# A-SHOJAEI/adverse-weather-semantic-segmentation-robustness-benchmark

Measured on AMD Instinct MI355X. Metric: images/sec (1024x2048, 5 weather conds, ensemble eval), higher is better.
Workload: dtype f32 (results float32; attention, gemm_1x1, winograd_3x3, segformer_head on 3xf16 split operands: 22-bit operands, f32 accumulate)

## Files before the change

### adverse_weather_semantic_segmentation_robustness_benchmark_amd/csrc/attn.hip

```cpp
#include "awseg_common.h"

namespace {

typedef float f32x16 __attribute__((ext_vector_type(16)));

constexpr int AT = 256;
#ifndef AWSEG_ATTN_SPLIT_WAVES
#define AWSEG_ATTN_SPLIT_WAVES 2
#endif
constexpr int D = 32;
constexpr int TK = 32;
constexpr int LDK = 36;

__device__ __forceinline__ constexpr int acc_row(int r, int hk) { return (r & 3) + 8 * (r >> 2) + 4 * hk; }

__global__ __launch_bounds__(AT, 2)
void attention_d32_kernel(const float* __restrict__ q, const float* __restrict__ k, const float* __restrict__ v,
                          float* __restrict__ out, int nq, int nkv, int heads, float scale_log2e, int kvp)
{
    __shared__ float sK[2][TK * LDK];
    __shared__ float sV[2][D * LDK];
    const int tid = threadIdx.x, lane = tid & 63, wave = tid >> 6;
    const int hk = lane >> 5, li = lane & 31;
    const int h = blockIdx.y, b = blockIdx.z;
    const int C = heads * D;
    const int q0 = blockIdx.x * 128 + wave * 32;
    const float* kb = k + (size_t)b * nkv * kvp + h * D;
    const float* vb = v + (size_t)b * nkv * kvp + h * D;

    float qf[16];
    {
        const int qi = q0 + li;
        const float* qp = q + ((size_t)b * nq + (qi < nq ? qi : nq - 1)) * C + h * D;
#pragma unroll
        for (int s4 = 0; s4 < 8; ++s4) {
            const float4 t4 = *reinterpret_cast<const float4*>(qp + 4 * s4);
            qf[2 * s4] = (hk ? t4.y : t4.x) * scale_log2e;
            qf[2 * s4 + 1] = (hk ? t4.w : t4.z) * scale_log2e;
        }
    }
    const int lkey = tid >> 3, lc = tid & 7;
    const size_t g_off = (size_t)lkey * kvp + 4 * lc;
    const int wk0 = lkey * LDK + 2 * lc;
    const int vkk = (lkey >> 2) & 1, vr = (lkey & 3) + 4 * (lkey >> 3);
    const int wv0 = (4 * lc) * LDK + vkk * 16 + vr;
    auto stage = [&](int buf, const float4& kk4, const float4& vv4) {
        *reinterpret_cast<float2*>(&sK[buf][wk0]) = make_float2(kk4.x, kk4.z);
        *reinterpret_cast<float2*>(&sK[buf][wk0 + 16]) = make_float2(kk4.y, kk4.w);
        sV[buf][wv0] = vv4.x; sV[buf][wv0 + LDK] = vv4.y; sV[buf][wv0 + 2 * LDK] = vv4.z; sV[buf][wv0 + 3 * LDK] = vv4.w;
    };
    const int ntiles = nkv / TK;
    float4 kreg = *reinterpret_cast<const float4*>(kb + g_off), vreg = *reinterpret_cast<const float4*>(vb + g_off);
    stage(0, kreg, vreg);
    if (ntiles > 1) {
        kreg = *reinterpret_cast<const float4*>(kb + (size_t)TK * kvp + g_off);
        vreg = *reinterpret_cast<const float4*>(vb + (size_t)TK * kvp + g_off);
    }
    __syncthreads();

    f32x16 oacc;
#pragma unroll
    for (int r = 0; r < 16; ++r) oacc[r] = 0.f;
    float m_run = -1e30f, l_run = 0.f;
    const int a_off = li * LDK + hk * 16;

    for (int t = 0; t < ntiles; ++t) {
        const int buf = t & 1;
        float kf[16];
#pragma unroll
        for (int j = 0; j < 4; ++j) {
            const float4 t4 = *reinterpret_cast<const float4*>(&sK[buf][a_off + 4 * j]);
            kf[4 * j] = t4.x; kf[4 * j + 1] = t4.y; kf[4 * j + 2] = t4.z; kf[4 * j + 3] = t4.w;
        }
        f32x16 sacc;
#pragma unroll
        for (int r = 0; r < 16; ++r) sacc[r] = 0.f;
#pragma unroll
        for (int s = 0; s < 16; ++s) sacc = __builtin_amdgcn_mfma_f32_32x32x2f32(kf[s], qf[s], sacc, 0, 0, 0);
        float vf[16];
#pragma unroll
        for (int j = 0; j < 4; ++j) {
            const float4 t4 = *reinterpret_cast<const float4*>(&sV[buf][a_off + 4 * j]);
            vf[4 * j] = t4.x; vf[4 * j + 1] = t4.y; vf[4 * j + 2] = t4.z; vf[4 * j + 3] = t4.w;
        }
        float mt = fmaxf(fmaxf(sacc[0], sacc[1]), fmaxf(sacc[2], sacc[3]));
#pragma unroll
        for (int r = 4; r < 16; r += 4) mt = fmaxf(mt, fmaxf(fmaxf(sacc[r], sacc[r + 1]), fmaxf(sacc[r + 2], sacc[r + 3])));
        mt = fmaxf(mt, __shfl_xor(mt, 32, 64));
        const float m_new = fmaxf(m_run, mt);
        const float alpha = __builtin_amdgcn_exp2f(m_run - m_new);
        float p[16], ls = 0.f;
#pragma unroll
        for (int r = 0; r < 16; ++r) { p[r] = __builtin_amdgcn_exp2f(sacc[r] - m_new); ls += p[r]; }
        ls += __shfl_xor(ls, 32, 64);
        l_run = l_run * alpha + ls;
        m_run = m_new;
        if (__builtin_amdgcn_ballot_w64(alpha != 1.0f) != 0) {
#pragma unroll
            for (int r = 0; r < 16; ++r) oacc[r] *= alpha;
        }
#pragma unroll
        for (int r = 0; r < 16; ++r) oacc = __builtin_amdgcn_mfma_f32_32x32x2f32(vf[r], p[r], oacc, 0, 0, 0);
        if (t + 1 < ntiles) {
            stage(buf ^ 1, kreg, vreg);
            if (t + 2 < ntiles) {
                kreg = *reinterpret_cast<const float4*>(kb + (size_t)(t + 2) * TK * kvp + g_off);
                vreg = *reinterpret_cast<const float4*>(vb + (size_t)(t + 2) * TK * kvp + g_off);
            }
        }
        __syncthreads();
    }

    const int qi = q0 + li;
    if (qi < nq) {
        const float inv = 1.0f / l_run;
        float* op = out + ((size_t)b * nq + qi) * C + h * D;
#pragma unroll
        for (int g = 0; g < 4; ++g)
            *reinterpret_cast<float4*>(op + 8 * g + 4 * hk) =
                make_float4(oacc[4 * g] * inv, oacc[4 * g + 1] * inv, oacc[4 * g + 2] * inv, oacc[4 * g + 3] * inv);
    }
}

typedef _Float16 h8 __attribute__((ext_vector_type(8)));
typedef _Float16 h2 __attribute__((ext_vector_type(2)));
typedef unsigned u32x4 __attribute__((ext_vector_type(4)));
typedef unsigned u32x2 __attribute__((ext_vector_type(2)));

constexpr int SROW = 72;
constexpr float kLoScale = 2048.0f, kLoInv = 1.0f / 2048.0f;

__device__ __forceinline__ void split_pair(float a, float b, unsigned& hi, unsigned& lo)
{
    const auto hp = __builtin_amdgcn_cvt_pkrtz(a, b);
    const h2 hh = __builtin_bit_cast(h2, hp);
    const float ra = (a - (float)hh.x) * kLoScale, rb = (b - (float)hh.y) * kLoScale;
    hi = __builtin_bit_cast(unsigned, hp);
    lo = __builtin_bit_cast(unsigned, __builtin_amdgcn_cvt_pkrtz(ra, rb));
}
__device__ __forceinline__ void split_pair_unscaled(float a, float b, unsigned& hi, unsigned& lo)
{
    hi = __builtin_bit_cast(unsigned, __builtin_amdgcn_cvt_pkrtz(a, b));
    asm("v_fma_mixlo_f16 %0, %1, 1.0, -%3 op_sel_hi:[0,0,1]\n\t"
        "v_fma_mixhi_f16 %0, %2, 1.0, -%3 op_sel:[0,0,1] op_sel_hi:[0,0,1]\n\t"
        "s_nop 1"
        : "=&v"(lo) : "v"(a), "v"(b), "v"(hi));
}
__device__ __forceinline__ void split8_unscaled(const float* x, h8& hi, h8& lo)
{
    u32x4 H, L;
#pragma unroll
    for (int i = 0; i < 4; ++i) { unsigned h, l; split_pair_unscaled(x[2 * i], x[2 * i + 1], h, l); H[i] = h; L[i] = l; }
    hi = __builtin_bit_cast(h8, H); lo = __builtin_bit_cast(h8, L);
}
__device__ __forceinline__ void split8(const float* x, h8& hi, h8& lo)
{
    u32x4 H, L;
#pragma unroll
    for (int i = 0; i < 4; ++i) { unsigned h, l; split_pair(x[2 * i], x[2 * i + 1], h, l); H[i] = h; L[i] = l; }
    hi = __builtin_bit_cast(h8, H); lo = __builtin_bit_cast(h8, L);
}
__device__ __forceinline__ constexpr int pv_slot(int key)
{
    return (key & 16) | (((key >> 2) & 1) << 3) | (((key >> 3) & 1) << 2) | (key & 3);
}

constexpr float kSplitLimit = 32768.0f;
struct attn_scales { float sq, sk, sv, bq, bk, bv; };

__device__ __forceinline__ float amax4(float m, const float4& t)
{
    m = __builtin_fmaxf(__builtin_fmaxf(m, __builtin_fabsf(t.x)), __builtin_fabsf(t.y));
    return __builtin_fmaxf(__builtin_fmaxf(m, __builtin_fabsf(t.z)), __builtin_fabsf(t.w));
}

typedef __bf16 bf8 __attribute__((ext_vector_type(8)));
__device__ __forceinline__ unsigned pack_bf16(float a, float b)
{
    typedef __bf16 bf2 __attribute__((ext_vector_type(2)));
    typedef float f2 __attribute__((ext_vector_type(2)));
    return __builtin_bit_cast(unsigned, __builtin_convertvector(f2{a, b}, bf2));
}
__device__ __forceinline__ h8 pack8_bf16(const float* x)
{
    u32x4 H;
#pragma unroll
    for (int i = 0; i < 4; ++i) H[i] = pack_bf16(x[2 * i], x[2 * i + 1]);
    return __builtin_bit_cast(h8, H);
}
#define MFMA_BF(A, B, C) __builtin_amdgcn_mfma_f32_32x32x16_bf16(__builtin_bit_cast(bf8, A), __builtin_bit_cast(bf8, B), C, 0, 0, 0)

template <bool SCALED, bool BF16 = false>
__device__ __forceinline__ bool attn_split_pass(const float* __restrict__ q, const float* __restrict__ k, const float* __restrict__ v,
                                                float* __restrict__ out, int nq, int nkv, int heads, float scale_log2e, int kvp,
                                                _Float16 (*sK)[TK * SROW], _Float16 (*sV)[D * SROW], unsigned* sMax, const attn_scales sc)
{
    const int tid = threadIdx.x, lane = tid & 63, wave = tid >> 6;
    const int hk = lane >> 5, li = lane & 31;
    const int h = blockIdx.y, b = blockIdx.z;
    const int C = heads * D;
    const int q0 = blockIdx.x * 128 + wave * 32;
    const float* kb = k + (size_t)b * nkv * kvp + h * D;
    const float* vb = v + (size_t)b * nkv * kvp + h * D;
    float qmax = 0.f, kmax = 0.f, vmax = 0.f;

    h8 qh[2], ql[2];
    {
        const int qi = q0 + li;
        const float* qp = q + ((size_t)b * nq + (qi < nq ? qi : nq - 1)) * C + h * D;
        const float qs = SCALED ? scale_log2e * sc.sq : scale_log2e;
#pragma unroll
        for (int s = 0; s < 2; ++s) {
            const float4 a4 = *reinterpret_cast<const float4*>(qp + 16 * s + 8 * hk);
            const float4 b4 = *reinterpret_cast<const float4*>(qp + 16 * s + 8 * hk + 4);
            const float x[8] = { a4.x * qs, a4.y * qs, a4.z * qs, a4.w * qs, b4.x * qs, b4.y * qs, b4.z * qs, b4.w * qs };
            if (BF16) { qh[s] = pack8_bf16(x); continue; }
            if (!SCALED) {
#pragma unroll
                for (int i = 0; i < 8; ++i) qmax = __builtin_fmaxf(qmax, __builtin_fabsf(x[i]));
            }
            split8(x, qh[s], ql[s]);
        }
    }
    const int lkey = tid >> 3, lc = tid & 7;
    const size_t g_off = (size_t)lkey * kvp + 4 * lc;
    const int wk0 = lkey * SROW + 4 * lc;
    const int wv0 = (4 * lc) * SROW + pv_slot(lkey);
    auto stage = [&](int buf, float4 kk4, float4 vv4) {
        if (BF16) {
            u32x2 H;
            H[0] = pack_bf16(kk4.x, kk4.y); H[1] = pack_bf16(kk4.z, kk4.w);
            *reinterpret_cast<u32x2*>(&sK[buf][wk0]) = H;
            const unsigned v01 = pack_bf16(vv4.x, vv4.y), v23 = pack_bf16(vv4.z, vv4.w);
            unsigned short* svb = reinterpret_cast<unsigned short*>(&sV[buf][wv0]);
            svb[0] = (unsigned short)v01; svb[SROW] = (unsigned short)(v01 >> 16);
            svb[2 * SROW] = (unsigned short)v23; svb[3 * SROW] = (unsigned short)(v23 >> 16);
            return;
        }
        if (SCALED) {
            kk4.x *= sc.sk; kk4.y *= sc.sk; kk4.z *= sc.sk; kk4.w *= sc.sk;
            vv4.x *= sc.sv; vv4.y *= sc.sv; vv4.z *= sc.sv; vv4.w *= sc.sv;
        } else {
            kmax = amax4(kmax, kk4); vmax = amax4(vmax, vv4);
        }
        u32x2 H, L; unsigned hh, ll;
        split_pair(kk4.x, kk4.y, hh, ll); H[0] = hh; L[0] = ll;
        split_pair(kk4.z, kk4.w, hh, ll); H[1] = hh; L[1] = ll;
        *reinterpret_cast<u32x2*>(&sK[buf][wk0]) = H;
        *reinterpret_cast<u32x2*>(&sK[buf][wk0 + 32]) = L;
        unsigned vh01, vl01, vh23, vl23;
        split_pair(vv4.x, vv4.y, vh01, vl01);
        split_pair(vv4.z, vv4.w, vh23, vl23);
        unsigned short* sv = reinterpret_cast<unsigned short*>(&sV[buf][wv0]);
        sv[0] = (unsigned short)vh01;            sv[32] = (unsigned short)vl01;
        sv[SROW] = (unsigned short)(vh01 >> 16); sv[SROW + 32] = (unsigned short)(vl01 >> 16);
        sv[2 * SROW] = (unsigned short)vh23;     sv[2 * SROW + 32] = (unsigned short)vl23;
        sv[3 * SROW] = (unsigned short)(vh23 >> 16); sv[3 * SROW + 32] = (unsigned short)(vl23 >> 16);
    };
    const int ntiles = nkv / TK;
    float4 kreg = *reinterpret_cast<const float4*>(kb + g_off), vreg = *reinterpret_cast<const float4*>(vb + g_off);
    stage(0, kreg, vreg);
    if (ntiles > 1) {
        kreg = *reinterpret_cast<const float4*>(kb + (size_t)TK * kvp + g_off);
        vreg = *reinterpret_cast<const float4*>(vb + (size_t)TK * kvp + g_off);
    }
    __syncthreads();

    f32x16 om, oc;
#pragma unroll
    for (int r = 0; r < 16; ++r) { om[r] = 0.f; oc[r] = 0.f; }
    float m_run = -1e30f, l_run = 0.f;
    const int a_off = li * SROW + 8 * hk;

    for (int t = 0; t < ntiles; ++t) {
        const int buf = t & 1;
        const h8* kr = reinterpret_cast<const h8*>(&sK[buf][a_off]);
        const h8 kh0 = kr[0], kh1 = kr[2], kl0 = kr[4], kl1 = kr[6];
        f32x16 sm, scx;
#pragma unroll
        for (int r = 0; r < 16; ++r) { sm[r] = 0.f; scx[r] = 0.f; }
        if (BF16) {
            sm = MFMA_BF(kh0, qh[0], sm);
            sm = MFMA_BF(kh1, qh[1], sm);
        } else {
            sm = __builtin_amdgcn_mfma_f32_32x32x16_f16(kh0, qh[0], sm, 0, 0, 0);
            scx = __builtin_amdgcn_mfma_f32_32x32x16_f16(kh0, ql[0], scx, 0, 0, 0);
            sm = __builtin_amdgcn_mfma_f32_32x32x16_f16(kh1, qh[1], sm, 0, 0, 0);
            scx = __builtin_amdgcn_mfma_f32_32x32x16_f16(kh1, ql[1], scx, 0, 0, 0);
            scx = __builtin_amdgcn_mfma_f32_32x32x16_f16(kl0, qh[0], scx, 0, 0, 0);
            scx = __builtin_amdgcn_mfma_f32_32x32x16_f16(kl1, qh[1], scx, 0, 0, 0);
        }
        const h8* vr = reinterpret_cast<const h8*>(&sV[buf][a_off]);
        const h8 vh0 = vr[0], vh1 = vr[2], vl0 = vr[4], vl1 = vr[6];
        float s[16];
#pragma unroll
        for (int r = 0; r < 16; ++r) {
            s[r] = fmaf(scx[r], kLoInv, sm[r]);
            if (SCALED) s[r] = s[r] * sc.bq * sc.bk;
        }
        float mt = fmaxf(fmaxf(s[0], s[1]), fmaxf(s[2], s[3]));
#pragma unroll
        for (int r = 4; r < 16; r += 4) mt = fmaxf(mt, fmaxf(fmaxf(s[r], s[r + 1]), fmaxf(s[r + 2], s[r + 3])));
        mt = fmaxf(mt, __shfl_xor(mt, 32, 64));
        const float m_new = fmaxf(m_run, mt);
        const float alpha = __builtin_amdgcn_exp2f(m_run - m_new);
        const float m_sh = m_new - 15.0f;
        float p[16], ls = 0.f;
#pragma unroll
        for (int r = 0; r < 16; ++r) { p[r] = __builtin_amdgcn_exp2f(s[r] - m_sh); ls += p[r]; }
        ls += __shfl_xor(ls, 32, 64);
        l_run = l_run * alpha + ls;
        m_run = m_new;
        if (__builtin_amdgcn_ballot_w64(alpha != 1.0f) != 0) {
#pragma unroll
            for (int r = 0; r < 16; ++r) { om[r] *= alpha; oc[r] *= alpha; }
        }
        if (BF16) {
            om = MFMA_BF(vh0, pack8_bf16(p), om);
            om = MFMA_BF(vh1, pack8_bf16(p + 8), om);
            if (t + 1 < ntiles) {
                stage(buf ^ 1, kreg, vreg);
                if (t + 2 < ntiles) {
                    kreg = *reinterpret_cast<const float4*>(kb + (size_t)(t + 2) * TK * kvp + g_off);
                    vreg = *reinterpret_cast<const float4*>(vb + (size_t)(t + 2) * TK * kvp + g_off);
                }
            }
            __syncthreads();
            continue;
        }
        h8 ph0, pl0, ph1, pl1;
        split8_unscaled(p, ph0, pl0);
        split8_unscaled(p + 8, ph1, pl1);
        om = __builtin_amdgcn_mfma_f32_32x32x16_f16(vh0, ph0, om, 0, 0, 0);
        oc = __builtin_amdgcn_mfma_f32_32x32x16_f16(vl0, ph0, oc, 0, 0, 0);
        om = __builtin_amdgcn_mfma_f32_32x32x16_f16(vh1, ph1, om, 0, 0, 0);
        oc = __builtin_amdgcn_mfma_f32_32x32x16_f16(vl1, ph1, oc, 0, 0, 0);
        om = __builtin_amdgcn_mfma_f32_32x32x16_f16(vh0, pl0, om, 0, 0, 0);
        om = __builtin_amdgcn_mfma_f32_32x32x16_f16(vh1, pl1, om, 0, 0, 0);
        if (t + 1 < ntiles) {
            stage(buf ^ 1, kreg, vreg);
            if (t + 2 < ntiles) {
                kreg = *reinterpret_cast<const float4*>(kb + (size_t)(t + 2) * TK * kvp + g_off);
                vreg = *reinterpret_cast<const float4*>(vb + (size_t)(t + 2) * TK * kvp + g_off);
            }
        }
        __syncthreads();
    }

    if (!SCALED && !BF16) {
        if (qmax >= kSplitLimit) atomicMax(&sMax[0], __builtin_bit_cast(unsigned, qmax));
        if (kmax >= kSplitLimit) atomicMax(&sMax[1], __builtin_bit_cast(unsigned, kmax));
        if (vmax >= kSplitLimit) atomicMax(&sMax[2], __builtin_bit_cast(unsigned, vmax));
        __syncthreads();
        if ((sMax[0] | sMax[1] | sMax[2]) != 0u) return true;
    }
    const int qi = q0 + li;
    if (qi < nq) {
        const float inv = 1.0f / l_run;
        float* op = out + ((size_t)b * nq + qi) * C + h * D;
#pragma unroll
        for (int g = 0; g < 4; ++g) {
            float4 o4 = make_float4(fmaf(oc[4 * g], kLoInv, om[4 * g]) * inv, fmaf(oc[4 * g + 1], kLoInv, om[4 * g + 1]) * inv,
                                    fmaf(oc[4 * g + 2], kLoInv, om[4 * g + 2]) * inv, fmaf(oc[4 * g + 3], kLoInv, om[4 * g + 3]) * inv);
            if (SCALED) { o4.x *= sc.bv; o4.y *= sc.bv; o4.z *= sc.bv; o4.w *= sc.bv; }
            *reinterpret_cast<float4*>(op + 8 * g + 4 * hk) = o4;
        }
    }
    return false;
}

__device__ __forceinline__ int guard_exponent(unsigned maxbits)
{
    const int ex = (int)(maxbits >> 23) & 0xff;
    if (maxbits == 0u || ex == 0xff) return 0;
    return ex - 127 - 13;
}

__global__ __launch_bounds__(AT, AWSEG_ATTN_SPLIT_WAVES)
void attention_d32_split_kernel(const float* __restrict__ q, const float* __restrict__ k, const float* __restrict__ v,
                                float* __restrict__ out, int nq, int nkv, int heads, float scale_log2e, int kvp)
{
    __shared__ __attribute__((aligned(16))) _Float16 sK[2][TK * SROW];
    __shared__ __attribute__((aligned(16))) _Float16 sV[2][D * SROW];
    __shared__ unsigned sMax[3];
    if (threadIdx.x < 3) sMax[threadIdx.x] = 0u;
    const attn_scales one = {1.f, 1.f, 1.f, 1.f, 1.f, 1.f};
    if (!attn_split_pass<false>(q, k, v, out, nq, nkv, heads, scale_log2e, kvp, sK, sV, sMax, one)) return;
    const int eq = guard_exponent(sMax[0]), ek = guard_exponent(sMax[1]), ev = guard_exponent(sMax[2]);
    auto p2 = [](int e) { return __builtin_bit_cast(float, (unsigned)(127 + e) << 23); };
    const attn_scales sc = {p2(-eq), p2(-ek), p2(-ev), p2(eq), p2(ek), p2(ev)};
    attn_split_pass<true>(q, k, v, out, nq, nkv, heads, scale_log2e, kvp, sK, sV, sMax, sc);
}

constexpr int IMG_TILE_HALFS = (TK + D) * SROW;

__device__ __forceinline__ uint32_t at_lds_addr(const void* p) { return (uint32_t)(uintptr_t)(__attribute__((address_space(3))) const void*)p; }
__device__ __forceinline__ void at_dma16(__amdgpu_buffer_rsrc_t rsrc, uint32_t voff, uint32_t soff, uint32_t lds_base)
{
    asm volatile("s_mov_b32 m0, %3\n\ts_nop 0\n\tbuffer_load_dwordx4 %0, %1, %2 offen lds" : : "v"(voff), "s"(rsrc), "s"(soff), "s"(lds_base) : "m0", "memory");
}

__global__ __launch_bounds__(AT)
void attn_kv_image_kernel(const float* __restrict__ k, const float* __restrict__ v, int kvp, int nkv, int heads,
                          _Float16* __restrict__ img, int* __restrict__ exps)
{
    __shared__ unsigned sM[2];
    const int tid = threadIdx.x, h = blockIdx.x, b = blockIdx.y;
    const float* kb = k + (size_t)b * nkv * kvp + h * D;
    const float* vb = v + (size_t)b * nkv * kvp + h * D;
    const int lkey = tid >> 3, lc = tid & 7;
    const size_t g_off = (size_t)lkey * kvp + 4 * lc;
    const int wk0 = lkey * SROW + 4 * lc;
    const int wv0 = TK * SROW + (4 * lc) * SROW + pv_slot(lkey);
    const int ntiles = nkv / TK;
    if (tid < 2) sM[tid] = 0u;
    __syncthreads();
    float kmax = 0.f, vmax = 0.f;
    for (int t = 0; t < ntiles; ++t) {
        kmax = amax4(kmax, *reinterpret_cast<const float4*>(kb + (size_t)t * TK * kvp + g_off));
        vmax = amax4(vmax, *reinterpret_cast<const float4*>(vb + (size_t)t * TK * kvp + g_off));
    }
    if (kmax >= kSplitLimit) atomicMax(&sM[0], __builtin_bit_cast(unsigned, kmax));
    if (vmax >= kSplitLimit) atomicMax(&sM[1], __builtin_bit_cast(unsigned, vmax));
    __syncthreads();
    const int ek = guard_exponent(sM[0]), ev = guard_exponent(sM[1]);
    auto p2 = [](int e) { return __builtin_bit_cast(float, (unsigned)(127 + e) << 23); };
    const float sk = p2(-ek), sv = p2(-ev);
    if (tid == 0) { exps[((size_t)b * heads + h) * 2] = ek; exps[((size_t)b * heads + h) * 2 + 1] = ev; }
    _Float16* base = img + ((size_t)b * heads + h) * ntiles * IMG_TILE_HALFS;
    for (int t = 0; t < ntiles; ++t) {
        float4 kk4 = *reinterpret_cast<const float4*>(kb + (size_t)t * TK * kvp + g_off);
        float4 vv4 = *reinterpret_cast<const float4*>(vb + (size_t)t * TK * kvp + g_off);
        kk4.x *= sk; kk4.y *= sk; kk4.z *= sk; kk4.w *= sk;
        vv4.x *= sv; vv4.y *= sv; vv4.z *= sv; vv4.w *= sv;
        _Float16* T = base + (size_t)t * IMG_TILE_HALFS;
        u32x2 H, L; unsigned hh, ll;
        split_pair(kk4.x, kk4.y, hh, ll); H[0] = hh; L[0] = ll;
        split_pair(kk4.z, kk4.w, hh, ll); H[1] = hh; L[1] = ll;
        *reinterpret_cast<u32x2*>(&T[wk0]) = H;
        *reinterpret_cast<u32x2*>(&T[wk0 + 32]) = L;
        unsigned vh01, vl01, vh23, vl23;
        split_pair(vv4.x, vv4.y, vh01, vl01);
        split_pair(vv4.z, vv4.w, vh23, vl23);
        unsigned short* sv16 = reinterpret_cast<unsigned short*>(&T[wv0]);
        sv16[0] = (unsigned short)vh01;            sv16[32] = (unsigned short)vl01;
        sv16[SROW] = (unsigned short)(vh01 >> 16); sv16[SROW + 32] = (unsigned short)(vl01 >> 16);
        sv16[2 * SROW] = (unsigned short)vh23;     sv16[2 * SROW + 32] = (unsigned short)vl23;
        sv16[3 * SROW] = (unsigned short)(vh23 >> 16); sv16[3 * SROW + 32] = (unsigned short)(vl23 >> 16);
    }
}

template <bool SCALED, bool QGUARD>
__device__ __forceinline__ bool attn_split_pass_img(const float* __restrict__ q, const _Float16* __restrict__ img_bh, float* __restrict__ out,
                                                    int nq, int nkv, int heads, float scale_log2e, _Float16 (*sKV)[IMG_TILE_HALFS],
                                                    unsigned* sMax, const attn_scales sc)
{
    const int tid = threadIdx.x, lane = tid & 63, wave = tid >> 6;
    const int hk = lane >> 5, li = lane & 31;
    const int h = blockIdx.y, b = blockIdx.z;
    const int C = heads * D;
    const int q0 = blockIdx.x * 128 + wave * 32;
    float qmax = 0.f;
    h8 qh[2], ql[2];
    {
        const int qi = q0 + li;
        const float* qp = q + ((size_t)b * nq + (qi < nq ? qi : nq - 1)) * C + h * D;
        const float qs = SCALED ? scale_log2e * sc.sq : scale_log2e;
#pragma unroll
        for (int s = 0; s < 2; ++s) {
            const float4 a4 = *reinterpret_cast<const float4*>(qp + 16 * s + 8 * hk);
            const float4 b4 = *reinterpret_cast<const float4*>(qp + 16 * s + 8 * hk + 4);
            const float x[8] = { a4.x * qs, a4.y * qs, a4.z * qs, a4.w * qs, b4.x * qs, b4.y * qs, b4.z * qs, b4.w * qs };
            if (QGUARD) {
#pragma unroll
                for (int i = 0; i < 8; ++i) qmax = __builtin_fmaxf(qmax, __builtin_fabsf(x[i]));
            }
            split8(x, qh[s], ql[s]);
        }
    }
    const int ntiles = nkv / TK;
    const __amdgpu_buffer_rsrc_t rsrc = __builtin_amdgcn_make_buffer_rsrc((void*)img_bh, 0, ntiles * IMG_TILE_HALFS * 2, 0x00020000);
    const uint32_t lds0 = __builtin_amdgcn_readfirstlane(at_lds_addr(&sKV[0][0]));
    const uint32_t wave_u = __builtin_amdgcn_readfirstlane(wave);
    auto dma_tile = [&](int t, int buf) {
        const uint32_t so = (uint32_t)t * (uint32_t)(IMG_TILE_HALFS * 2), lb = lds0 + (uint32_t)buf * (uint32_t)(IMG_TILE_HALFS * 2);
        at_dma16(rsrc, (uint32_t)(lane * 16) + wave_u * 1024u, so, lb + wave_u * 1024u);
        at_dma16(rsrc, (uint32_t)(lane * 16) + (wave_u + 4u) * 1024u, so, lb + (wave_u + 4u) * 1024u);
        if (wave_u == 0) at_dma16(rsrc, (uint32_t)(lane * 16) + 8192u, so, lb + 8192u);
    };
    dma_tile(0, 0);
    asm volatile("s_waitcnt vmcnt(0)" ::: "memory");
    __syncthreads();

    f32x16 om, oc;
#pragma unroll
    for (int r = 0; r < 16; ++r) { om[r] = 0.f; oc[r] = 0.f; }
    float m_run = -1e30f, l_run = 0.f;
    const int a_off = li * SROW + 8 * hk;

    for (int t = 0; t < ntiles; ++t) {
        const int buf = t & 1;
        if (t + 1 < ntiles) dma_tile(t + 1, buf ^ 1);
        const h8* kr = reinterpret_cast<const h8*>(&sKV[buf][a_off]);
        const h8 kh0 = kr[0], kh1 = kr[2], kl0 = kr[4], kl1 = kr[6];
        f32x16 sm, scx;
#pragma unroll
        for (int r = 0; r < 16; ++r) { sm[r] = 0.f; scx[r] = 0.f; }
        sm = __builtin_amdgcn_mfma_f32_32x32x16_f16(kh0, qh[0], sm, 0, 0, 0);
        scx = __builtin_amdgcn_mfma_f32_32x32x16_f16(kh0, ql[0], scx, 0, 0, 0);
        sm = __builtin_amdgcn_mfma_f32_32x32x16_f16(kh1, qh[1], sm, 0, 0, 0);
        scx = __builtin_amdgcn_mfma_f32_32x32x16_f16(kh1, ql[1], scx, 0, 0, 0);
        scx = __builtin_amdgcn_mfma_f32_32x32x16_f16(kl0, qh[0], scx, 0, 0, 0);
        scx = __builtin_amdgcn_mfma_f32_32x32x16_f16(kl1, qh[1], scx, 0, 0, 0);
        const h8* vr = reinterpret_cast<const h8*>(&sKV[buf][TK * SROW + a_off]);
        const h8 vh0 = vr[0], vh1 = vr[2], vl0 = vr[4], vl1 = vr[6];
        float s[16];
#pragma unroll
        for (int r = 0; r < 16; ++r) {
            s[r] = fmaf(scx[r], kLoInv, sm[r]);
            if (SCALED) s[r] = s[r] * sc.bq * sc.bk;
        }
        float mt = fmaxf(fmaxf(s[0], s[1]), fmaxf(s[2], s[3]));
#pragma unroll
        for (int r = 4; r < 16; r += 4) mt = fmaxf(mt, fmaxf(fmaxf(s[r], s[r + 1]), fmaxf(s[r + 2], s[r + 3])));
        mt = fmaxf(mt, __shfl_xor(mt, 32, 64));
        const float m_new = fmaxf(m_run, mt);
        const float alpha = __builtin_amdgcn_exp2f(m_run - m_new);
        const float m_sh = m_new - 15.0f;
        float p[16], ls = 0.f;
#pragma unroll
        for (int r = 0; r < 16; ++r) { p[r] = __builtin_amdgcn_exp2f(s[r] - m_sh); ls += p[r]; }
        ls += __shfl_xor(ls, 32, 64);
        l_run = l_run * alpha + ls;
        m_run = m_new;
        if (__builtin_amdgcn_ballot_w64(alpha != 1.0f) != 0) {
#pragma unroll
            for (int r = 0; r < 16; ++r) { om[r] *= alpha; oc[r] *= alpha; }
        }
        h8 ph0, pl0, ph1, pl1;
        split8_unscaled(p, ph0, pl0);
        split8_unscaled(p + 8, ph1, pl1);
        om = __builtin_amdgcn_mfma_f32_32x32x16_f16(vh0, ph0, om, 0, 0, 0);
        oc = __builtin_amdgcn_mfma_f32_32x32x16_f16(vl0, ph0, oc, 0, 0, 0);
        om = __builtin_amdgcn_mfma_f32_32x32x16_f16(vh1, ph1, om, 0, 0, 0);
        oc = __builtin_amdgcn_mfma_f32_32x32x16_f16(vl1, ph1, oc, 0, 0, 0);
        om = __builtin_amdgcn_mfma_f32_32x32x16_f16(vh0, pl0, om, 0, 0, 0);
        om = __builtin_amdgcn_mfma_f32_32x32x16_f16(vh1, pl1, om, 0, 0, 0);
        asm volatile("s_waitcnt vmcnt(0)" ::: "memory");
        __syncthreads();
    }

    if (QGUARD) {
        if (qmax >= kSplitLimit) atomicMax(&sMax[0], __builtin_bit_cast(unsigned, qmax));
        __syncthreads();
        if (sMax[0] != 0u) return true;
    }
    const int qi = q0 + li;
    if (qi < nq) {
        const float inv = 1.0f / l_run;
        float* op = out + ((size_t)b * nq + qi) * C + h * D;
#pragma unroll
        for (int g = 0; g < 4; ++g) {
            float4 o4 = make_float4(fmaf(oc[4 * g], kLoInv, om[4 * g]) * inv, fmaf(oc[4 * g + 1], kLoInv, om[4 * g + 1]) * inv,
                                    fmaf(oc[4 * g + 2], kLoInv, om[4 * g + 2]) * inv, fmaf(oc[4 * g + 3], kLoInv, om[4 * g + 3]) * inv);
            if (SCALED) { o4.x *= sc.bv; o4.y *= sc.bv; o4.z *= sc.bv; o4.w *= sc.bv; }
            *reinterpret_cast<float4*>(op + 8 * g + 4 * hk) = o4;
        }
    }
    return false;
}

__global__ __launch_bounds__(AT, AWSEG_ATTN_SPLIT_WAVES)
void attention_d32_split_img_kernel(const float* __restrict__ q, const _Float16* __restrict__ img, const int* __restrict__ exps,
                                    float* __restrict__ out, int nq, int nkv, int heads, float scale_log2e)
{
    __shared__ __attribute__((aligned(16))) _Float16 sKV[2][IMG_TILE_HALFS];
    __shared__ unsigned sMax[1];
    const int h = blockIdx.y, b = blockIdx.z;
    if (threadIdx.x == 0) sMax[0] = 0u;
    const _Float16* img_bh = img + ((size_t)b * heads + h) * (size_t)(nkv / TK) * IMG_TILE_HALFS;
    const int ek = exps[((size_t)b * heads + h) * 2], ev = exps[((size_t)b * heads + h) * 2 + 1];
    auto p2 = [](int e) { return __builtin_bit_cast(float, (unsigned)(127 + e) << 23); };
    attn_scales sc = {1.f, p2(-ek), p2(-ev), 1.f, p2(ek), p2(ev)};
    bool redo;
    if ((ek | ev) == 0) redo = attn_split_pass_img<false, true>(q, img_bh, out, nq, nkv, heads, scale_log2e, sKV, sMax, sc);
    else redo = attn_split_pass_img<true, true>(q, img_bh, out, nq, nkv, heads, scale_log2e, sKV, sMax, sc);
    if (!redo) return;
    const int eq = guard_exponent(sMax[0]);
    sc.sq = p2(-eq); sc.bq = p2(eq);
    __syncthreads();
    attn_split_pass_img<true, false>(q, img_bh, out, nq, nkv, heads, scale_log2e, sKV, sMax, sc);
}

__global__ __launch_bounds__(AT, 2)
void attention_d32_bf16_kernel(const float* __restrict__ q, const float* __restrict__ k, const float* __restrict__ v,
                               float* __restrict__ out, int nq, int nkv, int heads, float scale_log2e, int kvp)
{
    __shared__ __attribute__((aligned(16))) _Float16 sK[2][TK * SROW];
    __shared__ __attribute__((aligned(16))) _Float16 sV[2][D * SROW];
    __shared__ unsigned sMax[3];
    const attn_scales one = {1.f, 1.f, 1.f, 1.f, 1.f, 1.f};
    attn_split_pass<false, true>(q, k, v, out, nq, nkv, heads, scale_log2e, kvp, sK, sV, sMax, one);
}

}

namespace {
template <typename K>
int launch_attention(K kernel, const float* q, const float* k, const float* v, float* out, int batch, int heads,
                     int n_queries, int n_keys, float scale, awseg_stream_t stream, int kv_pitch = 0)
{
    if (batch == 0 || n_queries == 0) return 0;
    if (!q || !k || !v || !out || batch < 0 || heads < 1 || n_queries < 0 || n_keys < TK) return AWSEG_EINVAL;
    if (n_keys % TK) return AWSEG_ERANGE;
    if (heads > 65535 || batch > 65535) return AWSEG_ERANGE;
    if (((uintptr_t)q & 15) || ((uintptr_t)k & 15) || ((uintptr_t)v & 15) || ((uintptr_t)out & 15)) return AWSEG_EALIGN;
    if (kv_pitch == 0) kv_pitch = heads * D;
    if (kv_pitch < heads * D || (kv_pitch & 3)) return AWSEG_EINVAL;
    dim3 grid((unsigned)((n_queries + 127) / 128), (unsigned)heads, (unsigned)batch);
    hipLaunchKernelGGL(kernel, grid, dim3(AT), 0, awseg_s(stream), q, k, v, out, n_queries, n_keys, heads,
                       scale * 1.4426950408889634f, kv_pitch);
    AWSEG_LAUNCH_CHECK();
    return 0;
}
}

AWSEG_API int awseg_attention_d32(const float* q, const float* k, const float* v, float* out, int batch, int heads,
                                  int n_queries, int n_keys, float scale, awseg_stream_t stream)
{
    return launch_attention(attention_d32_kernel, q, k, v, out, batch, heads, n_queries, n_keys, scale, stream);
}

AWSEG_API int awseg_attention_d32_split(const float* q, const float* k, const float* v, float* out, int batch, int heads,
                                        int n_queries, int n_keys, float scale, awseg_stream_t stream)
{
    return launch_attention(attention_d32_split_kernel, q, k, v, out, batch, heads, n_queries, n_keys, scale, stream);
}

AWSEG_API int awseg_attention_d32_bf16(const float* q, const float* k, const float* v, float* out, int batch, int heads,
                                       int n_queries, int n_keys, float scale, awseg_stream_t stream)
{
    return launch_attention(attention_d32_bf16_kernel, q, k, v, out, batch, heads, n_queries, n_keys, scale, stream);
}

AWSEG_API int64_t awseg_attention_d32_split_workspace(int batch, int heads, int n_keys)
{
    if (batch < 0 || heads < 0 || n_keys < 0) return 0;
    const int64_t tab = ((int64_t)batch * heads * 2 * 4 + 255) / 256 * 256;
    return tab + (int64_t)batch * heads * (n_keys / TK) * IMG_TILE_HALFS * 2;
}

AWSEG_API int awseg_attention_d32_split_ws(const float* q, const float* k, const float* v, int kv_pitch, float* out, int batch, int heads,
                                           int n_queries, int n_keys, float scale, void* workspace, awseg_stream_t stream)
{
    if (batch == 0 || n_queries == 0) return 0;
    if (!q || !k || !v || !out || !workspace || batch < 0 || heads < 1 || n_queries < 0 || n_keys < TK) return AWSEG_EINVAL;
    if (n_keys % TK) return AWSEG_ERANGE;
    if (heads > 65535 || batch > 65535) return AWSEG_ERANGE;
    if (((uintptr_t)q & 15) || ((uintptr_t)k & 15) || ((uintptr_t)v & 15) || ((uintptr_t)out & 15) || ((uintptr_t)workspace & 255)) return AWSEG_EALIGN;
    if (kv_pitch == 0) kv_pitch = heads * D;
    if (kv_pitch < heads * D || (kv_pitch & 3)) return AWSEG_EINVAL;
    if ((int64_t)(n_keys / TK) * IMG_TILE_HALFS * 2 > 0x7fffffff) return AWSEG_ERANGE;
    int* exps = reinterpret_cast<int*>(workspace);
    const int64_t tab = ((int64_t)batch * heads * 2 * 4 + 255) / 256 * 256;
    _Float16* img = reinterpret_cast<_Float16*>(reinterpret_cast<char*>(workspace) + tab);
    hipLaunchKernelGGL(attn_kv_image_kernel, dim3((unsigned)heads, (unsigned)batch), dim3(AT), 0, awseg_s(stream), k, v, kv_pitch, n_keys, heads, img, exps);
    AWSEG_LAUNCH_CHECK();
    dim3 grid((unsigned)((n_queries + 127) / 128), (unsigned)heads, (unsigned)batch);
    hipLaunchKernelGGL(attention_d32_split_img_kernel, grid, dim3(AT), 0, awseg_s(stream), q, img, exps, out, n_queries, n_keys, heads,
                       scale * 1.4426950408889634f);
    AWSEG_LAUNCH_CHECK();
    return 0;
}

AWSEG_API int awseg_attention_d32_packed_kv(const float* q, const float* kv, float* out, int batch, int heads, int n_queries,
                                            int n_keys, float scale, int mode, awseg_stream_t stream)
{
    if (!kv) return AWSEG_EINVAL;
    const int c = heads * D;
    switch (mode) {
    case 0: return launch_attention(attention_d32_kernel, q, kv, kv + c, out, batch, heads, n_queries, n_keys, scale, stream, 2 * c);
    case 1: return launch_attention(attention_d32_split_kernel, q, kv, kv + c, out, batch, heads, n_queries, n_keys, scale, stream, 2 * c);
    case 2: return launch_attention(attention_d32_bf16_kernel, q, kv, kv + c, out, batch, heads, n_queries, n_keys, scale, stream, 2 * c);
    default: return AWSEG_EINVAL;
    }
}
```

Measured before the change: 227.7.

## Use stale integer-shifted running max in split attention softmax

Replaces the per-tile online-softmax max update with a lazily updated integer running max. The max is folded into the QK score accumulation as an extra MFMA with a ones vector, so the subtraction is free and rescaling happens only when scores exceed a threshold, using exact power-of-two alphas. This removes the per-tile cross-lane max and sum shuffles and most of the alpha rescaling. It adds one MFMA per tile and a fallback pass when the running max goes out of range, which doubles work in that rare case.

```diff
diff --git a/adverse_weather_semantic_segmentation_robustness_benchmark_amd/csrc/attn.hip b/adverse_weather_semantic_segmentation_robustness_benchmark_amd/csrc/attn.hip
--- a/adverse_weather_semantic_segmentation_robustness_benchmark_amd/csrc/attn.hip
+++ b/adverse_weather_semantic_segmentation_robustness_benchmark_amd/csrc/attn.hip
@@ -160,6 +160,55 @@
     for (int i = 0; i < 4; ++i) { unsigned h, l; split_pair(x[2 * i], x[2 * i + 1], h, l); H[i] = h; L[i] = l; }
     hi = __builtin_bit_cast(h8, H); lo = __builtin_bit_cast(h8, L);
 }
+constexpr float kTau = 4.0f;
+constexpr float kPre = 15.0f - kTau;
+constexpr float kStaleLimit = 2048.0f;
+struct stale_max { float m, l; u32x4 mb; bool oor; };
+__device__ __forceinline__ h8 stale_ones() { u32x4 o = {0x3c00u, 0u, 0u, 0u}; asm volatile("" : "+v"(o)); return __builtin_bit_cast(h8, o); }
+__device__ __forceinline__ unsigned stale_slice(float m, int hk)
+{
+    return __builtin_bit_cast(unsigned, __builtin_amdgcn_cvt_pkrtz(hk ? kPre : -m, 0.f));
+}
+__device__ __forceinline__ void stale_init(stale_max& st, int hk)
+{
+    st.m = 0.f; st.l = 0.f; st.oor = false;
+    st.mb = u32x4{stale_slice(0.f, hk), 0u, 0u, 0u};
+    asm volatile("" : "+v"(st.mb));
+}
+__device__ __forceinline__ void stale_softmax(const f32x16& sm, const f32x16& scx, bool first, int hk, stale_max& st, f32x16& om, f32x16& oc, float* p)
+{
+    float s[16];
+#pragma unroll
+    for (int r = 0; r < 16; ++r) s[r] = fmaf(scx[r], kLoInv, sm[r]);
+    float mt = fmaxf(fmaxf(s[0], s[1]), fmaxf(s[2], s[3]));
+#pragma unroll
+    for (int r = 4; r < 16; r += 4) mt = fmaxf(mt, fmaxf(fmaxf(s[r], s[r + 1]), fmaxf(s[r + 2], s[r + 3])));
+    if (first || __builtin_amdgcn_ballot_w64(mt > 15.0f) != 0) {
+        mt = fmaxf(mt, __shfl_xor(mt, 32, 64));
+        float d = __builtin_ceilf(mt - kPre);
+        if (!first) d = fmaxf(d, 0.f);
+        float mn = st.m + d;
+        if (!(__builtin_fabsf(mn) <= kStaleLimit)) {
+            st.oor = true;
+            mn = st.m; d = 0.f;
+        }
+        if (!first) {
+            const float alpha = __builtin_ldexpf(1.0f, -(int)d);
+#pragma unroll
+            for (int r = 0; r < 16; ++r) { om[r] *= alpha; oc[r] *= alpha; }
+            st.l *= alpha;
+        }
+        st.m = mn;
+        st.mb[0] = stale_slice(mn, hk);
+#pragma unroll
+        for (int r = 0; r < 16; ++r) s[r] -= d;
+    }
+    float ls = p[0] = __builtin_amdgcn_exp2f(s[0]);
+#pragma unroll
+    for (int r = 1; r < 16; ++r) { p[r] = __builtin_amdgcn_exp2f(s[r]); ls += p[r]; }
+    st.l += ls;
+}
+
 __device__ __forceinline__ constexpr int pv_slot(int key)
 {
     return (key & 16) | (((key >> 2) & 1) << 3) | (((key >> 3) & 1) << 2) | (key & 3);
@@ -190,7 +239,7 @@
 }
 #define MFMA_BF(A, B, C) __builtin_amdgcn_mfma_f32_32x32x16_bf16(__builtin_bit_cast(bf8, A), __builtin_bit_cast(bf8, B), C, 0, 0, 0)
 
-template <bool SCALED, bool BF16 = false>
+template <bool SCALED, bool BF16 = false, bool STALE = false>
 __device__ __forceinline__ bool attn_split_pass(const float* __restrict__ q, const float* __restrict__ k, const float* __restrict__ v,
                                                 float* __restrict__ out, int nq, int nkv, int heads, float scale_log2e, int kvp,
                                                 _Float16 (*sK)[TK * SROW], _Float16 (*sV)[D * SROW], unsigned* sMax, const attn_scales sc)
@@ -270,6 +319,9 @@
 #pragma unroll
     for (int r = 0; r < 16; ++r) { om[r] = 0.f; oc[r] = 0.f; }
     float m_run = -1e30f, l_run = 0.f;
+    stale_max st;
+    stale_init(st, hk);
+    const h8 ones = stale_ones();
     const int a_off = li * SROW + 8 * hk;
 
     for (int t = 0; t < ntiles; ++t) {
@@ -279,6 +331,7 @@
         f32x16 sm, scx;
 #pragma unroll
         for (int r = 0; r < 16; ++r) { sm[r] = 0.f; scx[r] = 0.f; }
+        if (STALE) sm = __builtin_amdgcn_mfma_f32_32x32x16_f16(ones, __builtin_bit_cast(h8, st.mb), sm, 0, 0, 0);
         if (BF16) {
             sm = MFMA_BF(kh0, qh[0], sm);
             sm = MFMA_BF(kh1, qh[1], sm);
@@ -292,28 +345,33 @@
         }
         const h8* vr = reinterpret_cast<const h8*>(&sV[buf][a_off]);
         const h8 vh0 = vr[0], vh1 = vr[2], vl0 = vr[4], vl1 = vr[6];
-        float s[16];
-#pragma unroll
-        for (int r = 0; r < 16; ++r) {
-            s[r] = fmaf(scx[r], kLoInv, sm[r]);
-            if (SCALED) s[r] = s[r] * sc.bq * sc.bk;
-        }
-        float mt = fmaxf(fmaxf(s[0], s[1]), fmaxf(s[2], s[3]));
-#pragma unroll
-        for (int r = 4; r < 16; r += 4) mt = fmaxf(mt, fmaxf(fmaxf(s[r], s[r + 1]), fmaxf(s[r + 2], s[r + 3])));
-        mt = fmaxf(mt, __shfl_xor(mt, 32, 64));
-        const float m_new = fmaxf(m_run, mt);
-        const float alpha = __builtin_amdgcn_exp2f(m_run - m_new);
-        const float m_sh = m_new - 15.0f;
-        float p[16], ls = 0.f;
-#pragma unroll
-        for (int r = 0; r < 16; ++r) { p[r] = __builtin_amdgcn_exp2f(s[r] - m_sh); ls += p[r]; }
-        ls += __shfl_xor(ls, 32, 64);
-        l_run = l_run * alpha + ls;
-        m_run = m_new;
-        if (__builtin_amdgcn_ballot_w64(alpha != 1.0f) != 0) {
-#pragma unroll
-            for (int r = 0; r < 16; ++r) { om[r] *= alpha; oc[r] *= alpha; }
+        float p[16];
+        if (STALE) {
+            stale_softmax(sm, scx, t == 0, hk, st, om, oc, p);
+        } else {
+            float s[16];
+#pragma unroll
+            for (int r = 0; r < 16; ++r) {
+                s[r] = fmaf(scx[r], kLoInv, sm[r]);
+                if (SCALED) s[r] = s[r] * sc.bq * sc.bk;
+            }
+            float mt = fmaxf(fmaxf(s[0], s[1]), fmaxf(s[2], s[3]));
+#pragma unroll
+            for (int r = 4; r < 16; r += 4) mt = fmaxf(mt, fmaxf(fmaxf(s[r], s[r + 1]), fmaxf(s[r + 2], s[r + 3])));
+            mt = fmaxf(mt, __shfl_xor(mt, 32, 64));
+            const float m_new = fmaxf(m_run, mt);
+            const float alpha = __builtin_amdgcn_exp2f(m_run - m_new);
+            const float m_sh = m_new - 15.0f;
+            float ls = 0.f;
+#pragma unroll
+            for (int r = 0; r < 16; ++r) { p[r] = __builtin_amdgcn_exp2f(s[r] - m_sh); ls += p[r]; }
+            ls += __shfl_xor(ls, 32, 64);
+            l_run = l_run * alpha + ls;
+            m_run = m_new;
+            if (__builtin_amdgcn_ballot_w64(alpha != 1.0f) != 0) {
+#pragma unroll
+                for (int r = 0; r < 16; ++r) { om[r] *= alpha; oc[r] *= alpha; }
+            }
         }
         if (BF16) {
             om = MFMA_BF(vh0, pack8_bf16(p), om);
@@ -351,9 +409,12 @@
         if (qmax >= kSplitLimit) atomicMax(&sMax[0], __builtin_bit_cast(unsigned, qmax));
         if (kmax >= kSplitLimit) atomicMax(&sMax[1], __builtin_bit_cast(unsigned, kmax));
         if (vmax >= kSplitLimit) atomicMax(&sMax[2], __builtin_bit_cast(unsigned, vmax));
+        if (STALE && st.oor) sMax[3] = 1u;
         __syncthreads();
         if ((sMax[0] | sMax[1] | sMax[2]) != 0u) return true;
-    }
+        if (STALE && sMax[3] != 0u) return true;
+    }
+    if (STALE) l_run = st.l + __shfl_xor(st.l, 32, 64);
     const int qi = q0 + li;
     if (qi < nq) {
         const float inv = 1.0f / l_run;
@@ -382,10 +443,14 @@
 {
     __shared__ __attribute__((aligned(16))) _Float16 sK[2][TK * SROW];
     __shared__ __attribute__((aligned(16))) _Float16 sV[2][D * SROW];
-    __shared__ unsigned sMax[3];
-    if (threadIdx.x < 3) sMax[threadIdx.x] = 0u;
+    __shared__ unsigned sMax[4];
+    if (threadIdx.x < 4) sMax[threadIdx.x] = 0u;
     const attn_scales one = {1.f, 1.f, 1.f, 1.f, 1.f, 1.f};
-    if (!attn_split_pass<false>(q, k, v, out, nq, nkv, heads, scale_log2e, kvp, sK, sV, sMax, one)) return;
+    if (!attn_split_pass<false, false, true>(q, k, v, out, nq, nkv, heads, scale_log2e, kvp, sK, sV, sMax, one)) return;
+    if ((sMax[0] | sMax[1] | sMax[2]) == 0u) {
+        attn_split_pass<false>(q, k, v, out, nq, nkv, heads, scale_log2e, kvp, sK, sV, sMax, one);
+        return;
+    }
     const int eq = guard_exponent(sMax[0]), ek = guard_exponent(sMax[1]), ev = guard_exponent(sMax[2]);
     auto p2 = [](int e) { return __builtin_bit_cast(float, (unsigned)(127 + e) << 23); };
     const attn_scales sc = {p2(-eq), p2(-ek), p2(-ev), p2(eq), p2(ek), p2(ev)};
@@ -450,7 +515,7 @@
     }
 }
 
-template <bool SCALED, bool QGUARD>
+template <bool SCALED, bool QGUARD, bool STALE>
 __device__ __forceinline__ bool attn_split_pass_img(const float* __restrict__ q, const _Float16* __restrict__ img_bh, float* __restrict__ out,
                                                     int nq, int nkv, int heads, float scale_log2e, _Float16 (*sKV)[IMG_TILE_HALFS],
                                                     unsigned* sMax, const attn_scales sc)
@@ -496,6 +561,9 @@
 #pragma unroll
     for (int r = 0; r < 16; ++r) { om[r] = 0.f; oc[r] = 0.f; }
     float m_run = -1e30f, l_run = 0.f;
+    stale_max st;
+    stale_init(st, hk);
+    const h8 ones = stale_ones();
     const int a_off = li * SROW + 8 * hk;
 
     for (int t = 0; t < ntiles; ++t) {
@@ -506,6 +574,7 @@
         f32x16 sm, scx;
 #pragma unroll
         for (int r = 0; r < 16; ++r) { sm[r] = 0.f; scx[r] = 0.f; }
+        if (STALE) sm = __builtin_amdgcn_mfma_f32_32x32x16_f16(ones, __builtin_bit_cast(h8, st.mb), sm, 0, 0, 0);
         sm = __builtin_amdgcn_mfma_f32_32x32x16_f16(kh0, qh[0], sm, 0, 0, 0);
         scx = __builtin_amdgcn_mfma_f32_32x32x16_f16(kh0, ql[0], scx, 0, 0, 0);
         sm = __builtin_amdgcn_mfma_f32_32x32x16_f16(kh1, qh[1], sm, 0, 0, 0);
@@ -514,28 +583,33 @@
         scx = __builtin_amdgcn_mfma_f32_32x32x16_f16(kl1, qh[1], scx, 0, 0, 0);
         const h8* vr = reinterpret_cast<const h8*>(&sKV[buf][TK * SROW + a_off]);
         const h8 vh0 = vr[0], vh1 = vr[2], vl0 = vr[4], vl1 = vr[6];
-        float s[16];
-#pragma unroll
-        for (int r = 0; r < 16; ++r) {
-            s[r] = fmaf(scx[r], kLoInv, sm[r]);
-            if (SCALED) s[r] = s[r] * sc.bq * sc.bk;
-        }
-        float mt = fmaxf(fmaxf(s[0], s[1]), fmaxf(s[2], s[3]));
-#pragma unroll
-        for (int r = 4; r < 16; r += 4) mt = fmaxf(mt, fmaxf(fmaxf(s[r], s[r + 1]), fmaxf(s[r + 2], s[r + 3])));
-        mt = fmaxf(mt, __shfl_xor(mt, 32, 64));
-        const float m_new = fmaxf(m_run, mt);
-        const float alpha = __builtin_amdgcn_exp2f(m_run - m_new);
-        const float m_sh = m_new - 15.0f;
-        float p[16], ls = 0.f;
-#pragma unroll
-        for (int r = 0; r < 16; ++r) { p[r] = __builtin_amdgcn_exp2f(s[r] - m_sh); ls += p[r]; }
-        ls += __shfl_xor(ls, 32, 64);
-        l_run = l_run * alpha + ls;
-        m_run = m_new;
-        if (__builtin_amdgcn_ballot_w64(alpha != 1.0f) != 0) {
-#pragma unroll
-            for (int r = 0; r < 16; ++r) { om[r] *= alpha; oc[r] *= alpha; }
+        float p[16];
+        if (STALE) {
+            stale_softmax(sm, scx, t == 0, hk, st, om, oc, p);
+        } else {
+            float s[16];
+#pragma unroll
+            for (int r = 0; r < 16; ++r) {
+                s[r] = fmaf(scx[r], kLoInv, sm[r]);
+                if (SCALED) s[r] = s[r] * sc.bq * sc.bk;
+            }
+            float mt = fmaxf(fmaxf(s[0], s[1]), fmaxf(s[2], s[3]));
+#pragma unroll
+            for (int r = 4; r < 16; r += 4) mt = fmaxf(mt, fmaxf(fmaxf(s[r], s[r + 1]), fmaxf(s[r + 2], s[r + 3])));
+            mt = fmaxf(mt, __shfl_xor(mt, 32, 64));
+            const float m_new = fmaxf(m_run, mt);
+            const float alpha = __builtin_amdgcn_exp2f(m_run - m_new);
+            const float m_sh = m_new - 15.0f;
+            float ls = 0.f;
+#pragma unroll
+            for (int r = 0; r < 16; ++r) { p[r] = __builtin_amdgcn_exp2f(s[r] - m_sh); ls += p[r]; }
+            ls += __shfl_xor(ls, 32, 64);
+            l_run = l_run * alpha + ls;
+            m_run = m_new;
+            if (__builtin_amdgcn_ballot_w64(alpha != 1.0f) != 0) {
+#pragma unroll
+                for (int r = 0; r < 16; ++r) { om[r] *= alpha; oc[r] *= alpha; }
+            }
         }
         h8 ph0, pl0, ph1, pl1;
         split8_unscaled(p, ph0, pl0);
@@ -552,9 +626,12 @@
 
     if (QGUARD) {
         if (qmax >= kSplitLimit) atomicMax(&sMax[0], __builtin_bit_cast(unsigned, qmax));
+        if (STALE && st.oor) sMax[1] = 1u;
         __syncthreads();
         if (sMax[0] != 0u) return true;
-    }
+        if (STALE && sMax[1] != 0u) return true;
+    }
+    if (STALE) l_run = st.l + __shfl_xor(st.l, 32, 64);
     const int qi = q0 + li;
     if (qi < nq) {
         const float inv = 1.0f / l_run;
@@ -575,21 +652,25 @@
                                     float* __restrict__ out, int nq, int nkv, int heads, float scale_log2e)
 {
     __shared__ __attribute__((aligned(16))) _Float16 sKV[2][IMG_TILE_HALFS];
-    __shared__ unsigned sMax[1];
+    __shared__ unsigned sMax[2];
     const int h = blockIdx.y, b = blockIdx.z;
-    if (threadIdx.x == 0) sMax[0] = 0u;
+    if (threadIdx.x < 2) sMax[threadIdx.x] = 0u;
     const _Float16* img_bh = img + ((size_t)b * heads + h) * (size_t)(nkv / TK) * IMG_TILE_HALFS;
     const int ek = exps[((size_t)b * heads + h) * 2], ev = exps[((size_t)b * heads + h) * 2 + 1];
     auto p2 = [](int e) { return __builtin_bit_cast(float, (unsigned)(127 + e) << 23); };
     attn_scales sc = {1.f, p2(-ek), p2(-ev), 1.f, p2(ek), p2(ev)};
     bool redo;
-    if ((ek | ev) == 0) redo = attn_split_pass_img<false, true>(q, img_bh, out, nq, nkv, heads, scale_log2e, sKV, sMax, sc);
-    else redo = attn_split_pass_img<true, true>(q, img_bh, out, nq, nkv, heads, scale_log2e, sKV, sMax, sc);
+    if ((ek | ev) == 0) redo = attn_split_pass_img<false, true, true>(q, img_bh, out, nq, nkv, heads, scale_log2e, sKV, sMax, sc);
+    else redo = attn_split_pass_img<true, true, false>(q, img_bh, out, nq, nkv, heads, scale_log2e, sKV, sMax, sc);
     if (!redo) return;
+    __syncthreads();
+    if (sMax[0] == 0u) {
+        attn_split_pass_img<false, false, false>(q, img_bh, out, nq, nkv, heads, scale_log2e, sKV, sMax, sc);
+        return;
+    }
     const int eq = guard_exponent(sMax[0]);
     sc.sq = p2(-eq); sc.bq = p2(eq);
-    __syncthreads();
-    attn_split_pass_img<true, false>(q, img_bh, out, nq, nkv, heads, scale_log2e, sKV, sMax, sc);
+    attn_split_pass_img<true, false, false>(q, img_bh, out, nq, nkv, heads, scale_log2e, sKV, sMax, sc);
 }
 
 __global__ __launch_bounds__(AT, 2)
```

Result: faster. 230.3, median of 6 (+1.1%).
